# bupt-ai-cz/HIAST

Measured on AMD Instinct MI355X. Metric: self-training images/sec (fwd+bwd+pseudo-label) at 1024x512, higher is better.
Workload: dtype fp16

## Files before the change

hiast_amd/csrc/common.h:

```cpp
#pragma once
#include <hip/hip_runtime.h>
#include <hip/hip_bf16.h>
#include <hip/hip_fp16.h>
#include <stdint.h>

#include <type_traits>

#include "../../include/hiast_hip.h"

#define HIAST_WAVE 64

#define HIAST_CHECK_LAUNCH()                         \
    do {                                             \
        hipError_t e__ = hipGetLastError();          \
        if (e__ != hipSuccess) return (int)e__;      \
    } while (0)

static inline int hiast_fmt_planes(int fmt) { return fmt == HIAST_FMT_SPLIT_BF16 ? 2 : 1; }
static inline int hiast_fmt_ok(int fmt) { return fmt == HIAST_FMT_BF16 || fmt == HIAST_FMT_SPLIT_BF16 || fmt == HIAST_FMT_FP16; }

int hiast_cu_count();
int hiast_grid_cus();

namespace hiast {

template <class F>
static inline bool for_class_count(int C, F&& f)
{
    switch (C) {
        case 19: f(std::integral_constant<int, 19>{}); return true;
        case 16: f(std::integral_constant<int, 16>{}); return true;
        case 9:  f(std::integral_constant<int, 9>{});  return true;
        case 2:  f(std::integral_constant<int, 2>{});  return true;
        default: return false;
    }
}

typedef __attribute__((ext_vector_type(8))) __bf16 h_bf16x8;
typedef __attribute__((ext_vector_type(8))) _Float16 h_f16x8;
typedef __attribute__((ext_vector_type(4))) float h_f32x4;
typedef __attribute__((ext_vector_type(16))) float h_f32x16;

typedef __attribute__((address_space(3))) void* h_lds_ptr;
__device__ __forceinline__ void h_dma16(__amdgpu_buffer_rsrc_t rs, unsigned char* lds, int voff, int soff)
{
    __builtin_amdgcn_raw_ptr_buffer_load_lds(rs, (h_lds_ptr)lds, 16, voff, soff, 0, 0);
}
__device__ __forceinline__ int h_lds_off(int row, int chunk) { return row * 128 + ((chunk ^ ((row >> 1) & 7)) << 4); }

#ifndef HIAST_NT
#define HIAST_NT 1
#endif
__device__ __forceinline__ void h_store_f32(float* p, float v)
{
#if HIAST_NT
    __builtin_nontemporal_store(v, p);
#else
    *p = v;
#endif
}
typedef unsigned int h_u32x4 __attribute__((ext_vector_type(4)));
__device__ __forceinline__ void h_store16(void* p, unsigned a, unsigned b, unsigned c, unsigned d)
{
#if HIAST_NT
    __builtin_nontemporal_store((h_u32x4){a, b, c, d}, reinterpret_cast<h_u32x4*>(p));
#else
    *reinterpret_cast<uint4*>(p) = make_uint4(a, b, c, d);
#endif
}
__device__ __forceinline__ void h_store16(void* p, unsigned a, unsigned b, unsigned c, unsigned d, bool nt)
{
#if HIAST_NT
    if (nt) {
        __builtin_nontemporal_store((h_u32x4){a, b, c, d}, reinterpret_cast<h_u32x4*>(p));
        return;
    }
#endif
    *reinterpret_cast<uint4*>(p) = make_uint4(a, b, c, d);
}
#ifndef H_NT_MIN_MIB
#define H_NT_MIN_MIB 64
#endif
constexpr long long H_NT_MIN_BYTES = (long long)H_NT_MIN_MIB << 20;
#ifndef HIAST_NT_OUT
#define HIAST_NT_OUT 0
#endif
__device__ __forceinline__ void h_store16_out(void* p, unsigned a, unsigned b, unsigned c, unsigned d)
{
    h_store16(p, a, b, c, d, HIAST_NT_OUT != 0);
}
__device__ __forceinline__ void h_store_f32_out(float* p, float v)
{
#if HIAST_NT_OUT
    __builtin_nontemporal_store(v, p);
#else
    *p = v;
#endif
}
#ifndef HIAST_NT_RES
#define HIAST_NT_RES 0
#endif
__device__ __forceinline__ uint4 h_load16_once(const void* p)
{
#if HIAST_NT_RES
    const h_u32x4 v = __builtin_nontemporal_load(reinterpret_cast<const h_u32x4*>(p));
    return make_uint4(v.x, v.y, v.z, v.w);
#else
    return *reinterpret_cast<const uint4*>(p);
#endif
}

template <bool F16>
struct H16;

template <>
struct H16<false> {
    static __device__ __forceinline__ float lo(unsigned w) { return __uint_as_float(w << 16); }
    static __device__ __forceinline__ float hi(unsigned w) { return __uint_as_float(w & 0xFFFF0000u); }
    static __device__ __forceinline__ float dec(unsigned short h) { return __uint_as_float((unsigned)h << 16); }
    static __device__ __forceinline__ unsigned short enc(float v) { return __bfloat16_as_ushort(__float2bfloat16(v)); }
    static __device__ __forceinline__ unsigned pack(float a, float b) { return (unsigned)enc(a) | ((unsigned)enc(b) << 16); }
    template <class V>
    static __device__ __forceinline__ h_f32x4 mfma16(const V& a, const V& b, h_f32x4 c)
    {
        return __builtin_amdgcn_mfma_f32_16x16x32_bf16(__builtin_bit_cast(h_bf16x8, a), __builtin_bit_cast(h_bf16x8, b), c, 0, 0, 0);
    }
    template <class V>
    static __device__ __forceinline__ h_f32x16 mfma32(const V& a, const V& b, h_f32x16 c)
    {
        return __builtin_amdgcn_mfma_f32_32x32x16_bf16(__builtin_bit_cast(h_bf16x8, a), __builtin_bit_cast(h_bf16x8, b), c, 0, 0, 0);
    }
// ... 100 lines not shown
```

hiast_amd/csrc/conv_launch.h:

```cpp
#pragma once
#include <stdlib.h>

#include "common.h"

namespace hiast {

struct IGeo {
    int H, W, Ho, Wo, stride, dil;
};

}

struct ConvLaunch {
    const void* x = nullptr;
    const void* wp = nullptr;
    void* y = nullptr;
    const void* res = nullptr;
    const void* res_gate = nullptr;
    int gate_mask = 0;
    const float* gamma = nullptr;
    const float* beta = nullptr;
    const float* mean = nullptr;
    const float* var = nullptr;
    float eps = 0.0f;
    int relu = 0;
    int64_t M = 0;
    int K = 0, N = 0, taps = 1;
    hiast::IGeo geo = {0, 0, 0, 0, 1, 1};
    int fmt = HIAST_FMT_BF16;
    int out_f32 = 0;
    float* stats = nullptr;
    int stats_rows = 0;
    int stats_mode = 0;
    hipStream_t st = nullptr;

    int planes() const { return hiast_fmt_planes(fmt); }
    bool f16() const { return fmt == HIAST_FMT_FP16; }
};

enum class ConvFamily { XCONV, XCONV2, TILE_F16, TILE };

struct ConvRoute {
    ConvFamily family = ConvFamily::TILE;
    int BN = 0, BM = 0;
    bool half9 = false;
    int rows = 0;
};

static inline int conv_panel_streams(int64_t M, int NG, int panel_rows)
{
    static const int env_cus = [] { const char* e = getenv("HIAST_XCONV_CUS"); const int v = e ? atoi(e) : 0; return v >= 8 && v <= 256 ? v : 0; }();
    const long long npanel = (M + panel_rows - 1) / panel_rows;
    long long streams = (env_cus ? env_cus : hiast_grid_cus()) / NG / 8 * 8;
    if (streams < 8) streams = 8;
    if (streams > npanel) streams = (npanel + 7) / 8 * 8;
    return (int)streams;
}

ConvRoute ig_route(const ConvLaunch& c);
int hiast_igemm_launch(const ConvLaunch& c);
int hiast_igemm_launch_f16(const ConvLaunch& c, const ConvRoute& r);
int hiast_xconv_ok(const ConvLaunch& c);
int hiast_xconv_stats_rows(int64_t M, int N);
int hiast_xconv_launch(const ConvLaunch& c, const ConvRoute& r);
int hiast_xconv2_ok(const ConvLaunch& c);
int hiast_xconv2_launch(const ConvLaunch& c);
int hiast_gemm_nt_launch(const void* x, const float* w, void* y, int64_t M, int K, int N, int dtype, hipStream_t st);
```

hiast_amd/csrc/igemm.hip:

```cpp
#include "igemm_kernel.h"

namespace hiast {

template <int PL>
__device__ __forceinline__ size_t ig_wp_elem(int n, int t, int k, int taps, int KO)
{
    const size_t row = ((size_t)n * taps + t) * PL * KO;
    return PL == 2 ? row + (size_t)(k >> 5) * 64 + (k & 31) : row + k;
}

template <int PL, bool F16 = false>
__global__ __launch_bounds__(256) void pack_conv_weight_kernel(const float* __restrict__ w,
                                                               unsigned short* __restrict__ wp,
                                                               unsigned short* __restrict__ wpt, int N, int K, int taps,
                                                               int mode)
{
    const long long idx = (long long)blockIdx.x * 256 + threadIdx.x;
    if (idx >= (long long)N * taps * K) return;
    const int k = (int)(idx % K);
    const int t = (int)((idx / K) % taps);
    const int n = (int)(idx / ((long long)K * taps));
    const float v = w[((size_t)n * K + k) * taps + t];
    unsigned short h, l = 0;
    if (F16) h = H16<true>::enc(v);
// ... 122 lines not shown
__global__ __launch_bounds__(256) void from_planes_kernel(const unsigned short* __restrict__ p, float* __restrict__ x,
                                                          long long M, int C)
{
    const long long total8 = M * C / 8;
    for (long long i = (long long)blockIdx.x * 256 + threadIdx.x; i < total8; i += (long long)gridDim.x * 256) {
        const long long m = (i * 8) / C;
        const int c = (int)((i * 8) - m * C);
        const unsigned short* src = p + ig_elem<2>((size_t)m, c, C);
        const uint4 h = *reinterpret_cast<const uint4*>(src), l = *reinterpret_cast<const uint4*>(src + 32);
        const unsigned wh[4] = {h.x, h.y, h.z, h.w}, wl[4] = {l.x, l.y, l.z, l.w};
        float v[8];
#pragma unroll
        for (int q = 0; q < 4; ++q) {
            v[2 * q] = __uint_as_float(wh[q] << 16) + __uint_as_float(wl[q] << 16);
            v[2 * q + 1] = __uint_as_float(wh[q] & 0xFFFF0000u) + __uint_as_float(wl[q] & 0xFFFF0000u);
        }
        reinterpret_cast<float4*>(x)[2 * i] = make_float4(v[0], v[1], v[2], v[3]);
        reinterpret_cast<float4*>(x)[2 * i + 1] = make_float4(v[4], v[5], v[6], v[7]);
    }
}

}

struct IgEnv {
    int half;
    int bn;
    int ragged_off;
    int cosched0;
};
static const IgEnv& ig_env()
{
    static const IgEnv env = [] {
        IgEnv e;
        const char* v = getenv("HIAST_IGEMM_HALF");
        e.half = v ? (atoi(v) != 0) : -1;
        v = getenv("HIAST_IGEMM_BN");
        const int bn = v ? atoi(v) : 0;
        e.bn = (bn == 64 || bn == 128 || bn == 256) ? bn : 0;
        e.ragged_off = getenv("HIAST_IGEMM_RAGGED") != nullptr;
        v = getenv("HIAST_IGEMM_COSCHED");
        e.cosched0 = v && atoi(v) != 0;
        return e;
    }();
    return env;
}
static thread_local int ig_cosched_tls = -1, ig_half_tls = -1;
extern "C" int hiast_igemm_set_half(int v)
{
    const int prev = ig_half_tls;
    ig_half_tls = v < 0 ? -1 : (v != 0);
    return prev;
}
extern "C" int hiast_igemm_set_cosched(int on)
{
    const int prev = ig_cosched_tls;
    ig_cosched_tls = on < 0 ? -1 : (on != 0);
    return prev;
}
static int ig_half_forced() { return ig_half_tls >= 0 ? ig_half_tls : ig_env().half; }
static int ig_cosched() { return ig_cosched_tls >= 0 ? ig_cosched_tls : ig_env().cosched0; }

#ifndef IG_HALF_AUTO
#define IG_HALF_BLOCKS(M, N) ((((M) + 255) / 256) * (((N) % 256 == 0) ? (N) / 256 : (N) / 128))
#define IG_HALF_AUTO(M, K, N) (IG_HALF_BLOCKS(M, N) <= 64 || (IG_HALF_BLOCKS(M, N) <= 128 && !ig_cosched()))
#endif
static int ig_half_tile(int64_t M, int K, int N, int taps, int out_f32)
{
    if (taps != 1 || out_f32 || N % 128 != 0 || M < 4096) return 0;
    if (ig_half_forced() >= 0) return ig_half_forced();
    return IG_HALF_AUTO(M, K, N);
}
static int ig_half_tile9(int64_t M, int N, int PL, bool bn_relu_only)
{
    if (PL != 2 || !bn_relu_only || N % 128 != 0 || M < 4096) return 0;
    if (ig_half_forced() >= 0) return ig_half_forced();
    return IG_HALF_AUTO(M, 0, N);
}

ConvRoute ig_route(const ConvLaunch& c)
{
    ConvRoute r;
    if (c.stats_mode != 2 && hiast_xconv_ok(c)) {
        r.family = ConvFamily::XCONV;
        r.rows = hiast_xconv_stats_rows(c.M, c.N);
        return r;
    }
    if (c.stats_mode == 0 && !c.f16() && hiast_xconv2_ok(c)) {
        r.family = ConvFamily::XCONV2;
        return r;
    }
    r.family = c.f16() ? ConvFamily::TILE_F16 : ConvFamily::TILE;
    r.BN = (c.N % 256 == 0) ? 256 : ((c.N % 128 == 0) ? 128 : 64);
    const bool plain = !c.mean && !c.gamma && !c.res && !c.relu && !c.res_gate && c.stats_mode == 0;
    if (plain && !c.out_f32 && r.BN == 128 && c.N > 512 && !ig_env().ragged_off) r.BN = 256;
    if (const int v = ig_env().bn) {
        if (c.N % v == 0) r.BN = v;
    }
    r.half9 = c.taps == 9 && !c.out_f32 && c.geo.stride == 1 &&
              ig_half_tile9(c.M, c.N, c.planes(), c.mean && c.relu && !c.res && !c.res_gate && c.stats_mode == 0) != 0;
    const bool half = r.half9 || (c.geo.stride >= 0 && ig_half_tile(c.M, c.K, c.N, c.taps, c.out_f32) != 0);
    if (half) r.BN = 128;
    r.BM = half ? 128 : hiast::IG_BM;
    r.rows = (int)((c.M + r.BM - 1) / r.BM);
    return r;
}

int hiast_igemm_launch(const ConvLaunch& in)
{
    ConvLaunch c = in;
    if (c.stats_mode != 2) c.stats_mode = c.stats ? 1 : 0;
    const int H = c.geo.H, W = c.geo.W, stride = c.geo.stride, dil = c.geo.dil;
    if (!hiast_fmt_ok(c.fmt)) return HIAST_E_RANGE;
    const int planes = c.planes();
    if (c.stats_mode == 2) {
        if (!c.stats || !c.res || !c.mean || !c.var || planes != 1 || c.out_f32 || c.relu || c.res_gate || c.N % 8) return HIAST_E_RANGE;
    } else {
        if (c.stats && (planes != 1 || c.out_f32 || c.res || c.relu)) return HIAST_E_RANGE;
        if ((c.stats || c.res_gate) && c.mean) return HIAST_E_RANGE;
    }
    if (c.res_gate && (planes != 1 || !c.res || c.relu || c.out_f32 || (!c.gate_mask && (((uintptr_t)c.res_gate) & 15)))) return HIAST_E_RANGE;
    if (!c.x || !c.wp || !c.y || (c.mean && !c.var)) return HIAST_E_ARG;
    if (c.M <= 0 || c.K <= 0 || c.N <= 0) return HIAST_E_ARG;
    if ((planes != 1 && planes != 2) || (c.taps != 1 && c.taps != 9)) return HIAST_E_RANGE;
    if ((c.K * planes) % 64 != 0 || c.N % 64 != 0 || c.M > (1ll << 31) - 512) return HIAST_E_RANGE;
    if (c.out_f32 && c.res) return HIAST_E_RANGE;
    if ((((uintptr_t)c.x) | ((uintptr_t)c.wp) | ((uintptr_t)c.y) | ((uintptr_t)c.res)) & 15) return HIAST_E_RANGE;
    c.geo = {0, 0, 0, 0, 1, 1};
    size_t in_pix = (size_t)c.M;
    if (c.taps != 1 && stride == -2) {
        if (H <= 0 || W <= 0 || dil != 1 || planes != 1 || c.out_f32) return HIAST_E_ARG;
        const int Hs = (H - 1) / 2 + 1, Ws = (W - 1) / 2 + 1;
        if (c.M % ((int64_t)H * W) != 0) return HIAST_E_ARG;
        c.geo = {Hs, Ws, H, W, -2, 1};
        in_pix = (size_t)(c.M / ((int64_t)H * W)) * Hs * Ws;
    } else if (c.taps != 1) {
        if (H <= 0 || W <= 0 || stride <= 0 || dil <= 0) return HIAST_E_ARG;
        const int Ho = (H - 1) / stride + 1, Wo = (W - 1) / stride + 1;
        if (c.M % ((int64_t)Ho * Wo) != 0) return HIAST_E_ARG;
        c.geo = {H, W, Ho, Wo, stride, dil};
        in_pix = (size_t)(c.M / ((int64_t)Ho * Wo)) * H * W;
    }
    if (in_pix * planes * c.K * 2 >= (1ull << 31) || (size_t)c.N * c.taps * planes * c.K * 2 >= (1ull << 31)) return HIAST_E_RANGE;
    const ConvRoute r = ig_route(c);
    if (c.stats_mode != 0 && c.stats_rows != r.rows) return HIAST_E_ARG;
    switch (r.family) {
    case ConvFamily::XCONV: return hiast_xconv_launch(c, r);
    case ConvFamily::XCONV2: return hiast_xconv2_launch(c);
    case ConvFamily::TILE_F16: return hiast_igemm_launch_f16(c, r);
    case ConvFamily::TILE: break;
    }
    if (planes == 2) return c.out_f32 ? launch_igemm_t<2, true>(c, r) : launch_igemm_t<2, false>(c, r);
    return c.out_f32 ? launch_igemm_t<1, true>(c, r) : launch_igemm_t<1, false>(c, r);
}

extern "C" int hiast_igemm_dgrad_bn_stats(const void* dy, const void* wpt, void* da, int B, int H, int W, int Cin, int Cout,
                                          int taps, int dil, const void* bn_x, const float* gamma, const float* beta,
                                          const float* save_mean, const float* save_invstd, float* partial, int partial_rows,
                                          int fmt, hiast_stream_t stream)
{
    if (fmt != HIAST_FMT_BF16 && fmt != HIAST_FMT_FP16) return HIAST_E_RANGE;
    if (B <= 0 || H <= 0 || W <= 0) return HIAST_E_ARG;
    if (!bn_x || !save_mean || !save_invstd || !partial) return HIAST_E_ARG;
    if ((((uintptr_t)save_mean) | ((uintptr_t)save_invstd) | ((uintptr_t)gamma) | ((uintptr_t)beta)) & 15) return HIAST_E_RANGE;
    ConvLaunch c;
    c.x = dy; c.wp = wpt; c.y = da; c.res = bn_x;
    c.gamma = gamma; c.beta = beta; c.mean = save_mean; c.var = save_invstd;
    c.M = (int64_t)B * H * W; c.K = Cin; c.N = Cout; c.taps = taps;
// ... 267 lines not shown
```

hiast_amd/csrc/xconv.hip:

```cpp
#include <hip/hip_bf16.h>
#include <stdlib.h>

#include "conv_launch.h"

namespace hiast {

constexpr int XC_PANEL = 64;
constexpr int XC_STAGES = 3;
constexpr int XC_COLS = 512;

__device__ __forceinline__ h_bf16x8 xc_lds_read(unsigned addr)
{
    h_bf16x8 v;
    asm volatile("ds_read_b128 %0, %1" : "=v"(v) : "v"(addr));
    return v;
}
__device__ __forceinline__ void xc_lds_wait(h_bf16x8& a, h_bf16x8& b)
{
    asm volatile("s_waitcnt lgkmcnt(0)" : "+v"(a), "+v"(b));
}

__device__ __forceinline__ int xc_chan(int g, int b, int r) { return (b >> 1) * 32 + g * 8 + (b & 1) * 4 + r; }

template <int KC, bool BN, bool RES, bool RELU, bool GATE, bool STATS, bool F16 = false>
__global__ __launch_bounds__(512) void xconv_kernel(const unsigned short* __restrict__ X,
                                                    const unsigned short* __restrict__ Wp,
                                                    const float* __restrict__ gamma, const float* __restrict__ beta,
                                                    const float* __restrict__ mean, const float* __restrict__ var,
                                                    float eps, const unsigned short* __restrict__ R,
                                                    const unsigned char* __restrict__ Rg,
                                                    unsigned short* __restrict__ Y, int M, int N,
                                                    float* __restrict__ stats)
{
    constexpr int SL = KC / 64;
    constexpr int KS = KC / 32;
    constexpr int STAGE = XC_PANEL * KC * 2;
    __shared__ __attribute__((aligned(1024))) unsigned char smem[XC_STAGES * STAGE];
    __shared__ float s_sc[XC_COLS], s_sh[XC_COLS];

    const int tid = threadIdx.x, lane = tid & 63;
    const int wave = __builtin_amdgcn_readfirstlane(tid >> 6);
    const int g = lane >> 4, px = lane & 15;
    const int NG = N / XC_COLS;
    const int xcd = blockIdx.x & 7, slot = blockIdx.x >> 3;
    const int cg = slot % NG;
    const int nstream = (int)gridDim.x / NG;
    const int stream = (slot / NG) * 8 + xcd;
    const int n0 = cg * XC_COLS + wave * 64;
    const int npanel = (M + XC_PANEL - 1) / XC_PANEL;

    h_bf16x8 wr[4][KS];
#pragma unroll
    for (int b = 0; b < 4; ++b) {
        const unsigned short* wrow = Wp + (size_t)(n0 + xc_chan(px >> 2, b, px & 3)) * KC + g * 8;
#pragma unroll
        for (int s = 0; s < KS; ++s) wr[b][s] = *reinterpret_cast<const h_bf16x8*>(wrow + s * 32);
    }
#pragma unroll
    for (int b = 0; b < 4; ++b)
#pragma unroll
        for (int s = 0; s < KS; ++s) asm volatile("" : "+v"(wr[b][s]));
    if (BN) {
        for (int c = tid; c < XC_COLS; c += 512) {
            const int n = cg * XC_COLS + c;
            const float sc = (gamma ? gamma[n] : 1.0f) * (1.0f / sqrtf(var[n] + eps));
            s_sc[c] = sc;
            s_sh[c] = fmaf(-mean[n], sc, beta ? beta[n] : 0.0f);
        }
        __syncthreads();
    }

    constexpr int OOB = (int)0x80000000;
    const __amdgpu_buffer_rsrc_t xrs = __builtin_amdgcn_make_buffer_rsrc((void*)X, 0, (int)((size_t)M * KC * 2), 0x00020000);
    const int drow = wave * 8 + (lane >> 3);
    const int dchunk = ((lane & 7) ^ ((drow >> 1) & 7)) * 16;
    auto issue = [&](int p, int st) {
        const int m = p * XC_PANEL + drow;
        const int voff = (p < npanel && m < M) ? (int)((size_t)m * KC * 2) + dchunk : OOB;
        unsigned char* base = smem + st * STAGE + wave * 1024;
#pragma unroll
        for (int j = 0; j < SL; ++j) h_dma16(xrs, base + j * (XC_PANEL * 128), voff, j * 128);
    };

    const unsigned lds_base = (unsigned)(size_t)smem;
    float st1[STATS ? 16 : 1], st2[STATS ? 16 : 1];
#pragma unroll
    for (int q = 0; q < (STATS ? 16 : 1); ++q) { st1[q] = 0.f; st2[q] = 0.f; }

    issue(stream, 0);
    issue(stream + nstream, 1);
    int it = 0;
    for (int p = stream; p < npanel; p += nstream, ++it) {
        const int st = it % XC_STAGES;
        constexpr int NRES = RES ? (GATE ? 8 : 4) : 0;
        if (it == 0) asm volatile("s_waitcnt vmcnt(%0)\n\ts_barrier" ::"n"(SL) : "memory");
        else asm volatile("s_waitcnt vmcnt(%0)\n\ts_barrier" ::"n"(SL + 8 + NRES) : "memory");
        uint4 rres[RES ? 2 : 1][2];
        unsigned rgate[GATE ? 2 : 1][2];
        auto load_res = [&](int half) {
#pragma unroll
            for (int t = 0; t < 2; ++t) {
                const int m = p * XC_PANEL + half * 32 + t * 16 + px;
                const size_t row = (size_t)(m < M ? m : 0) * N + n0 + g * 8;
                rres[t][0] = h_load16_once(R + row);
                rres[t][1] = h_load16_once(R + row + 32);
                if (GATE) {
                    const unsigned char* gp = Rg + (size_t)(m < M ? m : 0) * (N >> 3) + ((n0 + g * 8) >> 3);
                    rgate[t][0] = gp[0];
                    rgate[t][1] = gp[4];
                }
            }
        };
        if (RES) load_res(0);
        issue(p + 2 * nstream, (it + 2) % XC_STAGES);
#pragma unroll
        for (int half = 0; half < 2; ++half) {
            if (RES && half == 1) load_res(1);
            h_f32x4 acc[2][4];
#pragma unroll
            for (int a = 0; a < 2; ++a)
#pragma unroll
                for (int b = 0; b < 4; ++b) acc[a][b] = (h_f32x4){0.f, 0.f, 0.f, 0.f};
            auto frag = [&](int s, int a) {
                return xc_lds_read(lds_base + (unsigned)(st * STAGE + (s >> 1) * (XC_PANEL * 128) +
                                                         h_lds_off(half * 32 + a * 16 + px, (s & 1) * 4 + g)));
            };
            constexpr bool DB = !(STATS || (BN && RES));
            h_bf16x8 xa[DB ? 2 : 1][2];
            xa[0][0] = frag(0, 0);
            xa[0][1] = frag(0, 1);
            xc_lds_wait(xa[0][0], xa[0][1]);
#pragma unroll
            for (int s = 0; s < KS; ++s) {
                constexpr int one = DB ? 1 : 0;
                if (DB && s + 1 < KS) {
                    xa[(s + 1) & one][0] = frag(s + 1, 0);
                    xa[(s + 1) & one][1] = frag(s + 1, 1);
                }
#pragma unroll
                for (int a = 0; a < 2; ++a)
#pragma unroll
                    for (int b = 0; b < 4; ++b)
                        acc[a][b] = H16<F16>::mfma16(wr[b][s], xa[s & one][a], acc[a][b]);
                if (s + 1 < KS) {
                    if (!DB) {
                        xa[0][0] = frag(s + 1, 0);
                        xa[0][1] = frag(s + 1, 1);
                    }
                    xc_lds_wait(xa[(s + 1) & one][0], xa[(s + 1) & one][1]);
                }
            }
#pragma unroll
            for (int a = 0; a < 2; ++a) {
                const int m = p * XC_PANEL + half * 32 + a * 16 + px;
                const bool ok = m < M;
                const size_t row = (size_t)(ok ? m : 0) * N + n0 + g * 8;
                const uint4 r0 = rres[RES ? a : 0][0], r1 = rres[RES ? a : 0][1];
                const unsigned gate0 = GATE ? rgate[GATE ? a : 0][0] : 0xFFu;
                const unsigned gate1 = GATE ? rgate[GATE ? a : 0][1] : 0xFFu;
                float o[16];
#pragma unroll
                for (int b = 0; b < 4; ++b)
#pragma unroll
                    for (int r = 0; r < 4; ++r) o[(b >> 1) * 8 + (b & 1) * 4 + r] = acc[a][b][r];
                if (BN) {
#pragma unroll
                    for (int hh = 0; hh < 2; ++hh) {
                        const int c = wave * 64 + hh * 32 + g * 8;
#pragma unroll
                        for (int q = 0; q < 8; q += 4) {
                            const float4 sc = *reinterpret_cast<const float4*>(&s_sc[c + q]);
                            const float4 sh = *reinterpret_cast<const float4*>(&s_sh[c + q]);
                            o[hh * 8 + q] = fmaf(o[hh * 8 + q], sc.x, sh.x);
                            o[hh * 8 + q + 1] = fmaf(o[hh * 8 + q + 1], sc.y, sh.y);
                            o[hh * 8 + q + 2] = fmaf(o[hh * 8 + q + 2], sc.z, sh.z);
                            o[hh * 8 + q + 3] = fmaf(o[hh * 8 + q + 3], sc.w, sh.w);
                        }
                    }
                }
                if (RES) {
                    const unsigned w0[4] = {r0.x, r0.y, r0.z, r0.w}, w1[4] = {r1.x, r1.y, r1.z, r1.w};
#pragma unroll
                    for (int q = 0; q < 4; ++q) {
                        float a0 = H16<F16>::lo(w0[q]), a1 = H16<F16>::hi(w0[q]);
                        float b0 = H16<F16>::lo(w1[q]), b1 = H16<F16>::hi(w1[q]);
                        if (GATE) {
                            a0 = ((gate0 >> (2 * q)) & 1u) ? a0 : 0.f;
                            a1 = ((gate0 >> (2 * q + 1)) & 1u) ? a1 : 0.f;
                            b0 = ((gate1 >> (2 * q)) & 1u) ? b0 : 0.f;
                            b1 = ((gate1 >> (2 * q + 1)) & 1u) ? b1 : 0.f;
                        }
                        o[2 * q] += a0;
                        o[2 * q + 1] += a1;
                        o[8 + 2 * q] += b0;
                        o[8 + 2 * q + 1] += b1;
                    }
                }
                if (RELU) {
#pragma unroll
                    for (int q = 0; q < 16; ++q) o[q] = o[q] > 0.f ? o[q] : 0.f;
                }
                unsigned pk[8];
                if (STATS && F16) {
#pragma unroll
                    for (int q = 0; q < 8; ++q) {
                        pk[q] = H16<F16>::pack(o[2 * q], o[2 * q + 1]);
                        if (ok) {
                            const float v0 = H16<F16>::lo(pk[q]), v1 = H16<F16>::hi(pk[q]);
                            st1[2 * q] += v0; st2[2 * q] = fmaf(v0, v0, st2[2 * q]);
                            st1[2 * q + 1] += v1; st2[2 * q + 1] = fmaf(v1, v1, st2[2 * q + 1]);
                        }
                        __builtin_amdgcn_sched_barrier(0);
                    }
                } else {
#pragma unroll
                    for (int q = 0; q < 8; ++q) pk[q] = H16<F16>::pack(o[2 * q], o[2 * q + 1]);
                    if (STATS && ok) {
#pragma unroll
                        for (int q = 0; q < 8; ++q) {
                            const float v0 = H16<F16>::lo(pk[q]), v1 = H16<F16>::hi(pk[q]);
                            st1[2 * q] += v0; st2[2 * q] = fmaf(v0, v0, st2[2 * q]);
                            st1[2 * q + 1] += v1; st2[2 * q + 1] = fmaf(v1, v1, st2[2 * q + 1]);
                        }
                    }
                }
                if (ok) {
                    h_store16_out(Y + row, pk[0], pk[1], pk[2], pk[3]);
                    h_store16_out(Y + row + 32, pk[4], pk[5], pk[6], pk[7]);
                }
            }
        }
    }
    if (STATS) {
#pragma unroll
        for (int q = 0; q < 16; ++q) {
#pragma unroll
            for (int o = 1; o < 16; o <<= 1) {
                st1[q] += __shfl_xor(st1[q], o, 64);
                st2[q] += __shfl_xor(st2[q], o, 64);
            }
        }
        if (px == 0) {
            float* d = stats + ((size_t)stream * N + n0 + g * 8) * 2;
#pragma unroll
            for (int q = 0; q < 8; ++q) {
                d[2 * q] = st1[q];
                d[2 * q + 1] = st2[q];
                d[64 + 2 * q] = st1[8 + q];
                d[64 + 2 * q + 1] = st2[8 + q];
            }
        }
    }
}

}

int hiast_xconv_ok(const ConvLaunch& c)
{
    const char* env = getenv("HIAST_XCONV");
    const bool has_bn = c.mean != nullptr, has_res = c.res != nullptr;
    if ((env && atoi(env) == 0) || c.planes() != 1 || c.taps != 1 || c.out_f32) return 0;
    if (c.K != 256 || c.N % hiast::XC_COLS != 0 || c.N > 2048) return 0;
    if (c.res_gate && (!c.gate_mask || !has_res || c.relu)) return 0;
    if (has_bn && has_res && !c.relu) return 0;
    if (c.stats_mode == 1 && (has_res || c.relu || has_bn)) return 0;
    if (c.M < 4096) return 0;
    return 1;
}

int hiast_xconv_stats_rows(int64_t M, int N)
{
    return conv_panel_streams(M, N / hiast::XC_COLS, hiast::XC_PANEL);
}

int hiast_xconv_launch(const ConvLaunch& c, const ConvRoute& r)
{
    using namespace hiast;
    const dim3 grid((unsigned)(r.rows * (c.N / XC_COLS)));
#define XK(BNF, RESF, RELUF, GATEF, STATSF, F16)                                                                      \
    hipLaunchKernelGGL((xconv_kernel<256, BNF, RESF, RELUF, GATEF, STATSF, F16>), grid, dim3(512), 0, c.st,           \
                       (const unsigned short*)c.x, (const unsigned short*)c.wp, c.gamma, c.beta, c.mean, c.var, c.eps, \
                       (const unsigned short*)c.res, (const unsigned char*)c.res_gate, (unsigned short*)c.y, (int)c.M, c.N, \
                       c.stats)
#define XL(BNF, RESF, RELUF, GATEF, STATSF)                                                                          \
    do {                                                                                                             \
        if (c.f16()) XK(BNF, RESF, RELUF, GATEF, STATSF, true);                                                      \
        else XK(BNF, RESF, RELUF, GATEF, STATSF, false);                                                             \
    } while (0)
    const bool bn = c.mean != nullptr;
    if (c.stats) { XL(false, false, false, false, true); }
    else if (c.res_gate) { XL(false, true, false, true, false); }
    else if (c.res) {
        if (bn) { if (c.relu) XL(true, true, true, false, false); else return HIAST_E_RANGE; }
        else { if (c.relu) XL(false, true, true, false, false); else XL(false, true, false, false, false); }
    } else {
        if (bn) { if (c.relu) XL(true, false, true, false, false); else XL(true, false, false, false, false); }
        else { if (c.relu) XL(false, false, true, false, false); else XL(false, false, false, false, false); }
    }
#undef XL
#undef XK
    HIAST_CHECK_LAUNCH();
    return 0;
}
```

hiast_amd/csrc/xconv_bs.hip:

```cpp
#include <hip/hip_bf16.h>
#include <stdlib.h>

#include "common.h"

namespace hiast {

constexpr int XB_PANEL = 64;
constexpr int XB_STAGES = 3;
constexpr int XB_COLS = 256;
constexpr int XB_KC = 256;

template <int IDX>
__device__ __forceinline__ h_bf16x8 xb_lds_read_i(unsigned addr)
{
    h_bf16x8 v;
    asm volatile("ds_read_b128 %0, %1 offset:%2" : "=v"(v) : "v"(addr), "i"(IDX * 2048));
    return v;
}
__device__ __forceinline__ h_bf16x8 xb_lds_read(unsigned addr, int idx)
{
    switch (idx) {
    case 1: return xb_lds_read_i<1>(addr);
    case 2: return xb_lds_read_i<2>(addr);
    case 3: return xb_lds_read_i<3>(addr);
    case 4: return xb_lds_read_i<4>(addr);
    case 5: return xb_lds_read_i<5>(addr);
    case 6: return xb_lds_read_i<6>(addr);
    case 7: return xb_lds_read_i<7>(addr);
    case 8: return xb_lds_read_i<8>(addr);
    case 9: return xb_lds_read_i<9>(addr);
    case 10: return xb_lds_read_i<10>(addr);
    case 11: return xb_lds_read_i<11>(addr);
    case 12: return xb_lds_read_i<12>(addr);
    case 13: return xb_lds_read_i<13>(addr);
    case 14: return xb_lds_read_i<14>(addr);
    case 15: return xb_lds_read_i<15>(addr);
    default: return xb_lds_read_i<0>(addr);
    }
}
__device__ __forceinline__ void xb_lds_wait(h_bf16x8& a, h_bf16x8& b)
{
    asm volatile("s_waitcnt lgkmcnt(0)" : "+v"(a), "+v"(b));
}

template <bool F16>
__global__ __launch_bounds__(512) void xconv_gated_bnstat_kernel(
    const unsigned short* __restrict__ X, const unsigned short* __restrict__ Wp, const unsigned short* __restrict__ R,
    const unsigned char* __restrict__ Rg, const unsigned short* __restrict__ BX, const unsigned char* __restrict__ BM,
    const float* __restrict__ bmean, const float* __restrict__ binvstd, unsigned short* __restrict__ Y, int M, int N,
    float* __restrict__ stats)
{
    constexpr int SL = XB_KC / 64;
    constexpr int KS = XB_KC / 32;
    constexpr int STAGE = XB_PANEL * XB_KC * 2;
    __shared__ __attribute__((aligned(1024))) unsigned char smem[XB_STAGES * STAGE];

    const int tid = threadIdx.x, lane = tid & 63;
    const int wave = __builtin_amdgcn_readfirstlane(tid >> 6);
    const int g = lane >> 4, px = lane & 15;
    const int NG = N / XB_COLS;
    const int xcd = blockIdx.x & 7, slot = blockIdx.x >> 3;
    const int cg = slot % NG;
    const int nstream = (int)gridDim.x / NG;
    const int stream = (slot / NG) * 8 + xcd;
    const int n0 = cg * XB_COLS + wave * 32;
    const int npanel = (M + XB_PANEL - 1) / XB_PANEL;
    const int c0 = n0 + g * 8;

    h_bf16x8 wr[2][KS];
#pragma unroll
    for (int b = 0; b < 2; ++b) {
        const unsigned short* wrow = Wp + (size_t)(n0 + (px >> 2) * 8 + b * 4 + (px & 3)) * XB_KC + g * 8;
#pragma unroll
        for (int s = 0; s < KS; ++s) wr[b][s] = *reinterpret_cast<const h_bf16x8*>(wrow + s * 32);
    }
#pragma unroll
    for (int b = 0; b < 2; ++b)
#pragma unroll
        for (int s = 0; s < KS; ++s) asm volatile("" : "+v"(wr[b][s]));

    constexpr int OOB = (int)0x80000000;
    const __amdgpu_buffer_rsrc_t xrs = __builtin_amdgcn_make_buffer_rsrc((void*)X, 0, (int)((size_t)M * XB_KC * 2), 0x00020000);
    const int drow = wave * 8 + (lane >> 3);
    const int dchunk = ((lane & 7) ^ ((drow >> 1) & 7)) * 16;
    auto issue = [&](int p, int st) {
        const int m = p * XB_PANEL + drow;
        const int voff = (p < npanel && m < M) ? (int)((size_t)m * XB_KC * 2) + dchunk : OOB;
        unsigned char* base = smem + st * STAGE + wave * 1024;
#pragma unroll
        for (int j = 0; j < SL; ++j) h_dma16(xrs, base + j * (XB_PANEL * 128), voff, j * 128);
    };
    const unsigned lds_base = (unsigned)(size_t)smem;
    float st1[8], st2[8];
#pragma unroll
    for (int q = 0; q < 8; ++q) { st1[q] = 0.f; st2[q] = 0.f; }

    struct Rows {
        uint4 res[4], bx[4];
        unsigned gate[4], bm[4];
    };
    Rows ring[2];
    auto load_rows = [&](Rows& r, int p) {
#pragma unroll
        for (int t = 0; t < 4; ++t) {
            const int m = p * XB_PANEL + t * 16 + px;
            const size_t mr = (size_t)((p < npanel && m < M) ? m : 0);
            r.res[t] = h_load16_once(R + mr * N + c0);
            r.gate[t] = Rg[mr * (N >> 3) + (c0 >> 3)];
            r.bx[t] = h_load16_once(BX + mr * N + c0);
            r.bm[t] = BM[mr * (N >> 3) + (c0 >> 3)];
        }
    };
    auto panel = [&](int p, int it, const Rows& cur, Rows& nxt) {
        const int st = it % XB_STAGES;
        if (it == 0) asm volatile("s_waitcnt vmcnt(%0)\n\ts_barrier" ::"n"(SL + 16) : "memory");
        else asm volatile("s_waitcnt vmcnt(%0)\n\ts_barrier" ::"n"(SL + 4) : "memory");
        load_rows(nxt, p + nstream);
        issue(p + 2 * nstream, (it + 2) % XB_STAGES);
        const unsigned fbase = lds_base + (unsigned)(st * STAGE) + (unsigned)h_lds_off(px, g);
#pragma unroll
        for (int half = 0; half < 2; ++half) {
            h_f32x4 acc[2][2];
#pragma unroll
            for (int a = 0; a < 2; ++a)
#pragma unroll
                for (int b = 0; b < 2; ++b) acc[a][b] = (h_f32x4){0.f, 0.f, 0.f, 0.f};
            auto frag = [&](int s, int a) {
                return xb_lds_read((s & 1) ? fbase ^ 64u : fbase, 4 * (s >> 1) + 2 * half + a);
            };
            h_bf16x8 xa[2][2];
            xa[0][0] = frag(0, 0);
            xa[0][1] = frag(0, 1);
            xb_lds_wait(xa[0][0], xa[0][1]);
#pragma unroll
            for (int s = 0; s < KS; ++s) {
                if (s + 1 < KS) {
                    xa[(s + 1) & 1][0] = frag(s + 1, 0);
                    xa[(s + 1) & 1][1] = frag(s + 1, 1);
                }
#pragma unroll
                for (int a = 0; a < 2; ++a)
#pragma unroll
                    for (int b = 0; b < 2; ++b) acc[a][b] = H16<F16>::mfma16(wr[b][s], xa[s & 1][a], acc[a][b]);
                if (s + 1 < KS) xb_lds_wait(xa[(s + 1) & 1][0], xa[(s + 1) & 1][1]);
            }
#pragma unroll
            for (int a = 0; a < 2; ++a) {
                const int t = 2 * half + a;
                const int m = p * XB_PANEL + t * 16 + px;
                const bool ok = m < M;
                const unsigned w0[4] = {cur.res[t].x, cur.res[t].y, cur.res[t].z, cur.res[t].w};
                const unsigned xw[4] = {cur.bx[t].x, cur.bx[t].y, cur.bx[t].z, cur.bx[t].w};
                const unsigned gate = cur.gate[t], bm = cur.bm[t];
                unsigned pk[4];
#pragma unroll
                for (int q = 0; q < 4; ++q) {
                    float o0 = acc[a][q >> 1][2 * (q & 1)], o1 = acc[a][q >> 1][2 * (q & 1) + 1];
                    o0 += ((gate >> (2 * q)) & 1u) ? H16<F16>::lo(w0[q]) : 0.f;
                    o1 += ((gate >> (2 * q + 1)) & 1u) ? H16<F16>::hi(w0[q]) : 0.f;
                    pk[q] = H16<F16>::pack(o0, o1);
                    if (ok) {
                        const float g0 = ((bm >> (2 * q)) & 1u) ? H16<F16>::lo(pk[q]) : 0.f;
                        const float g1 = ((bm >> (2 * q + 1)) & 1u) ? H16<F16>::hi(pk[q]) : 0.f;
                        st1[2 * q] += g0;
                        st2[2 * q] = fmaf(g0, H16<F16>::lo(xw[q]), st2[2 * q]);
                        st1[2 * q + 1] += g1;
                        st2[2 * q + 1] = fmaf(g1, H16<F16>::hi(xw[q]), st2[2 * q + 1]);
                    }
                }
                if (ok) h_store16_out(Y + (size_t)m * N + c0, pk[0], pk[1], pk[2], pk[3]);
            }
        }
    };

    issue(stream, 0);
    issue(stream + nstream, 1);
    load_rows(ring[0], stream);
    for (int p = stream, it = 0; p < npanel; p += 2 * nstream, it += 2) {
        panel(p, it, ring[0], ring[1]);
        if (p + nstream >= npanel) break;
        panel(p + nstream, it + 1, ring[1], ring[0]);
    }
#pragma unroll
    for (int q = 0; q < 8; ++q) {
#pragma unroll
        for (int o = 1; o < 16; o <<= 1) {
            st1[q] += __shfl_xor(st1[q], o, 64);
            st2[q] += __shfl_xor(st2[q], o, 64);
        }
    }
    if (px == 0) {
        float* d = stats + ((size_t)stream * N + c0) * 2;
#pragma unroll
        for (int q = 0; q < 8; ++q) {
            const float mu = bmean[c0 + q], is = binvstd[c0 + q];
            d[2 * q] = st1[q];
            d[2 * q + 1] = is * (st2[q] - mu * st1[q]);
        }
    }
}

static int xb_blocks(int64_t M, int N)
{
    const int NG = N / XB_COLS;
    const long long npanel = (M + XB_PANEL - 1) / XB_PANEL;
    long long streams = hiast_grid_cus() / NG / 8 * 8;
    if (streams < 8) streams = 8;
    if (streams > npanel) streams = (npanel + 7) / 8 * 8;
    return (int)(streams * NG);
}

// ... 36 lines not shown
```

Before: 143.7.

## Extend fused 1x1 xconv kernel to K=512 with narrower wave columns

Generalizes the persistent 1x1-conv (xconv) kernel so K=512 layers can use it. For K=512 it keeps one 32 KiB LDS stage per panel by halving the panel rows and using 32 output columns per wave. It also adds triple-buffered LDS fragment reads with counted waits and loads residual rows one panel ahead. This routes K=512 convs away from the generic igemm path, at the cost of more template instantiations and a register/occupancy profile that may not suit every shape.

```diff
diff --git a/hiast_amd/csrc/common.h b/hiast_amd/csrc/common.h
--- a/hiast_amd/csrc/common.h
+++ b/hiast_amd/csrc/common.h
@@ -47,6 +47,35 @@
     __builtin_amdgcn_raw_ptr_buffer_load_lds(rs, (h_lds_ptr)lds, 16, voff, soff, 0, 0);
 }
 __device__ __forceinline__ int h_lds_off(int row, int chunk) { return row * 128 + ((chunk ^ ((row >> 1) & 7)) << 4); }
+
+template <int IDX>
+__device__ __forceinline__ h_bf16x8 h_lds_read_2k_i(unsigned addr)
+{
+    h_bf16x8 v;
+    asm volatile("ds_read_b128 %0, %1 offset:%2" : "=v"(v) : "v"(addr), "i"(IDX * 2048));
+    return v;
+}
+__device__ __forceinline__ h_bf16x8 h_lds_read_2k(unsigned addr, int idx)
+{
+    switch (idx) {
+    case 1: return h_lds_read_2k_i<1>(addr);
+    case 2: return h_lds_read_2k_i<2>(addr);
+    case 3: return h_lds_read_2k_i<3>(addr);
+    case 4: return h_lds_read_2k_i<4>(addr);
+    case 5: return h_lds_read_2k_i<5>(addr);
+    case 6: return h_lds_read_2k_i<6>(addr);
+    case 7: return h_lds_read_2k_i<7>(addr);
+    case 8: return h_lds_read_2k_i<8>(addr);
+    case 9: return h_lds_read_2k_i<9>(addr);
+    case 10: return h_lds_read_2k_i<10>(addr);
+    case 11: return h_lds_read_2k_i<11>(addr);
+    case 12: return h_lds_read_2k_i<12>(addr);
+    case 13: return h_lds_read_2k_i<13>(addr);
+    case 14: return h_lds_read_2k_i<14>(addr);
+    case 15: return h_lds_read_2k_i<15>(addr);
+    default: return h_lds_read_2k_i<0>(addr);
+    }
+}
 
 #ifndef HIAST_NT
 #define HIAST_NT 1
diff --git a/hiast_amd/csrc/conv_launch.h b/hiast_amd/csrc/conv_launch.h
--- a/hiast_amd/csrc/conv_launch.h
+++ b/hiast_amd/csrc/conv_launch.h
@@ -61,7 +61,7 @@
 int hiast_igemm_launch(const ConvLaunch& c);
 int hiast_igemm_launch_f16(const ConvLaunch& c, const ConvRoute& r);
 int hiast_xconv_ok(const ConvLaunch& c);
-int hiast_xconv_stats_rows(int64_t M, int N);
+int hiast_xconv_stats_rows(int64_t M, int K, int N);
 int hiast_xconv_launch(const ConvLaunch& c, const ConvRoute& r);
 int hiast_xconv2_ok(const ConvLaunch& c);
 int hiast_xconv2_launch(const ConvLaunch& c);
diff --git a/hiast_amd/csrc/igemm.hip b/hiast_amd/csrc/igemm.hip
--- a/hiast_amd/csrc/igemm.hip
+++ b/hiast_amd/csrc/igemm.hip
@@ -228,7 +228,7 @@
     ConvRoute r;
     if (c.stats_mode != 2 && hiast_xconv_ok(c)) {
         r.family = ConvFamily::XCONV;
-        r.rows = hiast_xconv_stats_rows(c.M, c.N);
+        r.rows = hiast_xconv_stats_rows(c.M, c.K, c.N);
         return r;
     }
     if (c.stats_mode == 0 && !c.f16() && hiast_xconv2_ok(c)) {
diff --git a/hiast_amd/csrc/xconv.hip b/hiast_amd/csrc/xconv.hip
--- a/hiast_amd/csrc/xconv.hip
+++ b/hiast_amd/csrc/xconv.hip
@@ -5,9 +5,10 @@
 
 namespace hiast {
 
-constexpr int XC_PANEL = 64;
 constexpr int XC_STAGES = 3;
-constexpr int XC_COLS = 512;
+constexpr int XC_STAGE = 32768;
+constexpr int xc_cw(int K) { return K == 512 ? 32 : 64; }
+constexpr int xc_panel(int K) { return XC_STAGE / (K * 2); }
 
 __device__ __forceinline__ h_bf16x8 xc_lds_read(unsigned addr)
 {
@@ -15,14 +16,15 @@
     asm volatile("ds_read_b128 %0, %1" : "=v"(v) : "v"(addr));
     return v;
 }
+template <int LEFT = 0>
 __device__ __forceinline__ void xc_lds_wait(h_bf16x8& a, h_bf16x8& b)
 {
-    asm volatile("s_waitcnt lgkmcnt(0)" : "+v"(a), "+v"(b));
+    asm volatile("s_waitcnt lgkmcnt(%2)" : "+v"(a), "+v"(b) : "n"(LEFT));
 }
 
 __device__ __forceinline__ int xc_chan(int g, int b, int r) { return (b >> 1) * 32 + g * 8 + (b & 1) * 4 + r; }
 
-template <int KC, bool BN, bool RES, bool RELU, bool GATE, bool STATS, bool F16 = false>
+template <int KC, int CW, bool BN, bool RES, bool RELU, bool GATE, bool STATS, bool F16 = false>
 __global__ __launch_bounds__(512) void xconv_kernel(const unsigned short* __restrict__ X,
                                                     const unsigned short* __restrict__ Wp,
                                                     const float* __restrict__ gamma, const float* __restrict__ beta,
@@ -34,7 +36,14 @@
 {
     constexpr int SL = KC / 64;
     constexpr int KS = KC / 32;
+    constexpr int XC_PANEL = xc_panel(KC);
+    constexpr int XC_COLS = 8 * CW;
     constexpr int STAGE = XC_PANEL * KC * 2;
+    constexpr int NT = CW / 16;
+    constexpr int NQ = CW / 32;
+    constexpr int OC = 8 * NQ;
+    constexpr int HALVES = XC_PANEL / 32;
+    static_assert(STAGE == XC_STAGE && (CW == 64 || CW == 32) && (HALVES == 1 || HALVES == 2), "panel = one 32 KiB stage");
     __shared__ __attribute__((aligned(1024))) unsigned char smem[XC_STAGES * STAGE];
     __shared__ float s_sc[XC_COLS], s_sh[XC_COLS];
 
@@ -46,18 +55,18 @@
     const int cg = slot % NG;
     const int nstream = (int)gridDim.x / NG;
     const int stream = (slot / NG) * 8 + xcd;
-    const int n0 = cg * XC_COLS + wave * 64;
+    const int n0 = cg * XC_COLS + wave * CW;
     const int npanel = (M + XC_PANEL - 1) / XC_PANEL;
 
-    h_bf16x8 wr[4][KS];
-#pragma unroll
-    for (int b = 0; b < 4; ++b) {
+    h_bf16x8 wr[NT][KS];
+#pragma unroll
+    for (int b = 0; b < NT; ++b) {
         const unsigned short* wrow = Wp + (size_t)(n0 + xc_chan(px >> 2, b, px & 3)) * KC + g * 8;
 #pragma unroll
         for (int s = 0; s < KS; ++s) wr[b][s] = *reinterpret_cast<const h_bf16x8*>(wrow + s * 32);
     }
 #pragma unroll
-    for (int b = 0; b < 4; ++b)
+    for (int b = 0; b < NT; ++b)
 #pragma unroll
         for (int s = 0; s < KS; ++s) asm volatile("" : "+v"(wr[b][s]));
     if (BN) {
@@ -71,83 +80,126 @@
     }
 
     constexpr int OOB = (int)0x80000000;
+    constexpr int RG = XC_PANEL / 8;
+    constexpr int NDMA = SL * RG / 8;
+    static_assert(NDMA == 4, "the counted waits below assume 4 DMA instructions per wave and panel");
     const __amdgpu_buffer_rsrc_t xrs = __builtin_amdgcn_make_buffer_rsrc((void*)X, 0, (int)((size_t)M * KC * 2), 0x00020000);
-    const int drow = wave * 8 + (lane >> 3);
+    const int drg = RG == 8 ? wave : wave % RG, dsl = RG == 8 ? 0 : (wave / RG) * NDMA;
+    const int drow = drg * 8 + (lane >> 3);
     const int dchunk = ((lane & 7) ^ ((drow >> 1) & 7)) * 16;
     auto issue = [&](int p, int st) {
         const int m = p * XC_PANEL + drow;
         const int voff = (p < npanel && m < M) ? (int)((size_t)m * KC * 2) + dchunk : OOB;
-        unsigned char* base = smem + st * STAGE + wave * 1024;
-#pragma unroll
-        for (int j = 0; j < SL; ++j) h_dma16(xrs, base + j * (XC_PANEL * 128), voff, j * 128);
+        unsigned char* base = smem + st * STAGE + drg * 1024;
+#pragma unroll
+        for (int j = 0; j < NDMA; ++j) h_dma16(xrs, base + (dsl + j) * (XC_PANEL * 128), voff, (dsl + j) * 128);
     };
 
     const unsigned lds_base = (unsigned)(size_t)smem;
-    float st1[STATS ? 16 : 1], st2[STATS ? 16 : 1];
-#pragma unroll
-    for (int q = 0; q < (STATS ? 16 : 1); ++q) { st1[q] = 0.f; st2[q] = 0.f; }
+    float st1[STATS ? OC : 1], st2[STATS ? OC : 1];
+#pragma unroll
+    for (int q = 0; q < (STATS ? OC : 1); ++q) { st1[q] = 0.f; st2[q] = 0.f; }
+
+    auto load_rows = [&](int m0, auto& rr, auto& gg) {
+#pragma unroll
+        for (int t = 0; t < 2; ++t) {
+            const int m = m0 + t * 16 + px;
+            const size_t row = (size_t)(m < M ? m : 0) * N + n0 + g * 8;
+            rr[t][0] = h_load16_once(R + row);
+            if (NQ == 2) rr[t][1] = h_load16_once(R + row + 32);
+            if (GATE) {
+                const unsigned char* gp = Rg + (size_t)(m < M ? m : 0) * (N >> 3) + ((n0 + g * 8) >> 3);
+                gg[t][0] = gp[0];
+                if (NQ == 2) gg[t][1] = gp[4];
+            }
+        }
+    };
+    constexpr bool AHEAD = RES && HALVES == 1;
+    uint4 rnext[AHEAD ? 2 : 1][2];
+    unsigned gnext[AHEAD && GATE ? 2 : 1][2];
+    if (AHEAD) load_rows(stream * XC_PANEL, rnext, gnext);
 
     issue(stream, 0);
     issue(stream + nstream, 1);
     int it = 0;
     for (int p = stream; p < npanel; p += nstream, ++it) {
         const int st = it % XC_STAGES;
-        constexpr int NRES = RES ? (GATE ? 8 : 4) : 0;
-        if (it == 0) asm volatile("s_waitcnt vmcnt(%0)\n\ts_barrier" ::"n"(SL) : "memory");
-        else asm volatile("s_waitcnt vmcnt(%0)\n\ts_barrier" ::"n"(SL + 8 + NRES) : "memory");
+        constexpr int NRES = RES ? 2 * NQ * (GATE ? 2 : 1) : 0;
+        constexpr int NST = 2 * NQ;
+        if (it == 0) asm volatile("s_waitcnt vmcnt(%0)\n\ts_barrier" ::"n"(NDMA) : "memory");
+        else asm volatile("s_waitcnt vmcnt(%0)\n\ts_barrier" ::"n"(NDMA + HALVES * NST + (HALVES - 1) * NRES) : "memory");
         uint4 rres[RES ? 2 : 1][2];
         unsigned rgate[GATE ? 2 : 1][2];
-        auto load_res = [&](int half) {
+        auto load_res = [&](int half) { load_rows(p * XC_PANEL + half * 32, rres, rgate); };
+        if (AHEAD) {
 #pragma unroll
             for (int t = 0; t < 2; ++t) {
-                const int m = p * XC_PANEL + half * 32 + t * 16 + px;
-                const size_t row = (size_t)(m < M ? m : 0) * N + n0 + g * 8;
-                rres[t][0] = h_load16_once(R + row);
-                rres[t][1] = h_load16_once(R + row + 32);
-                if (GATE) {
-                    const unsigned char* gp = Rg + (size_t)(m < M ? m : 0) * (N >> 3) + ((n0 + g * 8) >> 3);
-                    rgate[t][0] = gp[0];
-                    rgate[t][1] = gp[4];
-                }
-            }
-        };
-        if (RES) load_res(0);
+                rres[t][0] = rnext[t][0];
+                if (GATE) rgate[t][0] = gnext[GATE ? t : 0][0];
+            }
+            load_rows((p + nstream) * XC_PANEL, rnext, gnext);
+        } else if (RES) load_res(0);
         issue(p + 2 * nstream, (it + 2) % XC_STAGES);
-#pragma unroll
-        for (int half = 0; half < 2; ++half) {
+        const unsigned fbase = lds_base + (unsigned)(st * STAGE) + (unsigned)h_lds_off(px, g);
+#pragma unroll
+        for (int half = 0; half < HALVES; ++half) {
             if (RES && half == 1) load_res(1);
-            h_f32x4 acc[2][4];
+            h_f32x4 acc[2][NT];
 #pragma unroll
             for (int a = 0; a < 2; ++a)
 #pragma unroll
-                for (int b = 0; b < 4; ++b) acc[a][b] = (h_f32x4){0.f, 0.f, 0.f, 0.f};
+                for (int b = 0; b < NT; ++b) acc[a][b] = (h_f32x4){0.f, 0.f, 0.f, 0.f};
             auto frag = [&](int s, int a) {
-                return xc_lds_read(lds_base + (unsigned)(st * STAGE + (s >> 1) * (XC_PANEL * 128) +
-                                                         h_lds_off(half * 32 + a * 16 + px, (s & 1) * 4 + g)));
+                if constexpr (HALVES == 1) return h_lds_read_2k((s & 1) ? fbase ^ 64u : fbase, 2 * (s >> 1) + a);
+                else return xc_lds_read(lds_base + (unsigned)(st * STAGE + (s >> 1) * (XC_PANEL * 128) +
+                                                              h_lds_off(half * 32 + a * 16 + px, (s & 1) * 4 + g)));
             };
-            constexpr bool DB = !(STATS || (BN && RES));
-            h_bf16x8 xa[DB ? 2 : 1][2];
-            xa[0][0] = frag(0, 0);
-            xa[0][1] = frag(0, 1);
-            xc_lds_wait(xa[0][0], xa[0][1]);
-#pragma unroll
-            for (int s = 0; s < KS; ++s) {
-                constexpr int one = DB ? 1 : 0;
-                if (DB && s + 1 < KS) {
-                    xa[(s + 1) & one][0] = frag(s + 1, 0);
-                    xa[(s + 1) & one][1] = frag(s + 1, 1);
-                }
-#pragma unroll
-                for (int a = 0; a < 2; ++a)
-#pragma unroll
-                    for (int b = 0; b < 4; ++b)
-                        acc[a][b] = H16<F16>::mfma16(wr[b][s], xa[s & one][a], acc[a][b]);
-                if (s + 1 < KS) {
-                    if (!DB) {
-                        xa[0][0] = frag(s + 1, 0);
-                        xa[0][1] = frag(s + 1, 1);
-                    }
-                    xc_lds_wait(xa[(s + 1) & one][0], xa[(s + 1) & one][1]);
+            constexpr bool DB = CW == 32 || !(STATS || (BN && RES));
+            if constexpr (CW == 32) {
+                h_bf16x8 xr[3][2];
+                xr[0][0] = frag(0, 0);
+                xr[0][1] = frag(0, 1);
+                xr[1][0] = frag(1, 0);
+                xr[1][1] = frag(1, 1);
+                xc_lds_wait<2>(xr[0][0], xr[0][1]);
+#pragma unroll
+                for (int s = 0; s < KS; ++s) {
+                    if (s + 2 < KS) {
+                        xr[(s + 2) % 3][0] = frag(s + 2, 0);
+                        xr[(s + 2) % 3][1] = frag(s + 2, 1);
+                    }
+#pragma unroll
+                    for (int a = 0; a < 2; ++a)
+#pragma unroll
+                        for (int b = 0; b < NT; ++b)
+                            acc[a][b] = H16<F16>::mfma16(wr[b][s], xr[s % 3][a], acc[a][b]);
+                    if (s + 2 < KS) xc_lds_wait<2>(xr[(s + 1) % 3][0], xr[(s + 1) % 3][1]);
+                    else if (s + 1 < KS) xc_lds_wait<0>(xr[(s + 1) % 3][0], xr[(s + 1) % 3][1]);
+                }
+            } else {
+                h_bf16x8 xa[DB ? 2 : 1][2];
+                xa[0][0] = frag(0, 0);
+                xa[0][1] = frag(0, 1);
+                xc_lds_wait(xa[0][0], xa[0][1]);
+#pragma unroll
+                for (int s = 0; s < KS; ++s) {
+                    constexpr int one = DB ? 1 : 0;
+                    if (DB && s + 1 < KS) {
+                        xa[(s + 1) & one][0] = frag(s + 1, 0);
+                        xa[(s + 1) & one][1] = frag(s + 1, 1);
+                    }
+#pragma unroll
+                    for (int a = 0; a < 2; ++a)
+#pragma unroll
+                        for (int b = 0; b < NT; ++b)
+                            acc[a][b] = H16<F16>::mfma16(wr[b][s], xa[s & one][a], acc[a][b]);
+                    if (s + 1 < KS) {
+                        if (!DB) {
+                            xa[0][0] = frag(s + 1, 0);
+                            xa[0][1] = frag(s + 1, 1);
+                        }
+                        xc_lds_wait(xa[(s + 1) & one][0], xa[(s + 1) & one][1]);
+                    }
                 }
             }
 #pragma unroll
@@ -155,18 +207,18 @@
                 const int m = p * XC_PANEL + half * 32 + a * 16 + px;
                 const bool ok = m < M;
                 const size_t row = (size_t)(ok ? m : 0) * N + n0 + g * 8;
-                const uint4 r0 = rres[RES ? a : 0][0], r1 = rres[RES ? a : 0][1];
+                const uint4 r0 = rres[RES ? a : 0][0], r1 = rres[RES ? a : 0][NQ - 1];
                 const unsigned gate0 = GATE ? rgate[GATE ? a : 0][0] : 0xFFu;
-                const unsigned gate1 = GATE ? rgate[GATE ? a : 0][1] : 0xFFu;
-                float o[16];
-#pragma unroll
-                for (int b = 0; b < 4; ++b)
+                const unsigned gate1 = GATE ? rgate[GATE ? a : 0][NQ - 1] : 0xFFu;
+                float o[OC];
+#pragma unroll
+                for (int b = 0; b < NT; ++b)
 #pragma unroll
                     for (int r = 0; r < 4; ++r) o[(b >> 1) * 8 + (b & 1) * 4 + r] = acc[a][b][r];
                 if (BN) {
 #pragma unroll
-                    for (int hh = 0; hh < 2; ++hh) {
-                        const int c = wave * 64 + hh * 32 + g * 8;
+                    for (int hh = 0; hh < NQ; ++hh) {
+                        const int c = wave * CW + hh * 32 + g * 8;
 #pragma unroll
                         for (int q = 0; q < 8; q += 4) {
                             const float4 sc = *reinterpret_cast<const float4*>(&s_sc[c + q]);
@@ -192,18 +244,20 @@
                         }
                         o[2 * q] += a0;
                         o[2 * q + 1] += a1;
-                        o[8 + 2 * q] += b0;
-                        o[8 + 2 * q + 1] += b1;
+                        if (NQ == 2) {
+                            o[OC - 8 + 2 * q] += b0;
+                            o[OC - 8 + 2 * q + 1] += b1;
+                        }
                     }
                 }
                 if (RELU) {
 #pragma unroll
-                    for (int q = 0; q < 16; ++q) o[q] = o[q] > 0.f ? o[q] : 0.f;
-                }
-                unsigned pk[8];
+                    for (int q = 0; q < OC; ++q) o[q] = o[q] > 0.f ? o[q] : 0.f;
+                }
+                unsigned pk[OC / 2];
                 if (STATS && F16) {
 #pragma unroll
-                    for (int q = 0; q < 8; ++q) {
+                    for (int q = 0; q < OC / 2; ++q) {
                         pk[q] = H16<F16>::pack(o[2 * q], o[2 * q + 1]);
                         if (ok) {
                             const float v0 = H16<F16>::lo(pk[q]), v1 = H16<F16>::hi(pk[q]);
@@ -214,10 +268,10 @@
                     }
                 } else {
 #pragma unroll
-                    for (int q = 0; q < 8; ++q) pk[q] = H16<F16>::pack(o[2 * q], o[2 * q + 1]);
+                    for (int q = 0; q < OC / 2; ++q) pk[q] = H16<F16>::pack(o[2 * q], o[2 * q + 1]);
                     if (STATS && ok) {
 #pragma unroll
-                        for (int q = 0; q < 8; ++q) {
+                        for (int q = 0; q < OC / 2; ++q) {
                             const float v0 = H16<F16>::lo(pk[q]), v1 = H16<F16>::hi(pk[q]);
                             st1[2 * q] += v0; st2[2 * q] = fmaf(v0, v0, st2[2 * q]);
                             st1[2 * q + 1] += v1; st2[2 * q + 1] = fmaf(v1, v1, st2[2 * q + 1]);
@@ -226,14 +280,14 @@
                 }
                 if (ok) {
                     h_store16_out(Y + row, pk[0], pk[1], pk[2], pk[3]);
-                    h_store16_out(Y + row + 32, pk[4], pk[5], pk[6], pk[7]);
+                    if (NQ == 2) h_store16_out(Y + row + 32, pk[OC / 2 - 4], pk[OC / 2 - 3], pk[OC / 2 - 2], pk[OC / 2 - 1]);
                 }
             }
         }
     }
     if (STATS) {
 #pragma unroll
-        for (int q = 0; q < 16; ++q) {
+        for (int q = 0; q < OC; ++q) {
 #pragma unroll
             for (int o = 1; o < 16; o <<= 1) {
                 st1[q] += __shfl_xor(st1[q], o, 64);
@@ -246,8 +300,10 @@
             for (int q = 0; q < 8; ++q) {
                 d[2 * q] = st1[q];
                 d[2 * q + 1] = st2[q];
-                d[64 + 2 * q] = st1[8 + q];
-                d[64 + 2 * q + 1] = st2[8 + q];
+                if (NQ == 2) {
+                    d[64 + 2 * q] = st1[OC - 8 + q];
+                    d[64 + 2 * q + 1] = st2[OC - 8 + q];
+                }
             }
         }
     }
@@ -260,7 +316,10 @@
     const char* env = getenv("HIAST_XCONV");
     const bool has_bn = c.mean != nullptr, has_res = c.res != nullptr;
     if ((env && atoi(env) == 0) || c.planes() != 1 || c.taps != 1 || c.out_f32) return 0;
-    if (c.K != 256 || c.N % hiast::XC_COLS != 0 || c.N > 2048) return 0;
+    if (c.K == 512) {
+        const char* e5 = getenv("HIAST_XCONV_K512");
+        if ((e5 && atoi(e5) == 0) || c.N % (8 * hiast::xc_cw(512)) != 0 || c.N < 2 * c.K) return 0;
+    } else if (c.K != 256 || c.N % (8 * hiast::xc_cw(256)) != 0 || c.N > 2048) return 0;
     if (c.res_gate && (!c.gate_mask || !has_res || c.relu)) return 0;
     if (has_bn && has_res && !c.relu) return 0;
     if (c.stats_mode == 1 && (has_res || c.relu || has_bn)) return 0;
@@ -268,24 +327,29 @@
     return 1;
 }
 
-int hiast_xconv_stats_rows(int64_t M, int N)
-{
-    return conv_panel_streams(M, N / hiast::XC_COLS, hiast::XC_PANEL);
+int hiast_xconv_stats_rows(int64_t M, int K, int N)
+{
+    return conv_panel_streams(M, N / (8 * hiast::xc_cw(K)), hiast::xc_panel(K));
 }
 
 int hiast_xconv_launch(const ConvLaunch& c, const ConvRoute& r)
 {
     using namespace hiast;
-    const dim3 grid((unsigned)(r.rows * (c.N / XC_COLS)));
-#define XK(BNF, RESF, RELUF, GATEF, STATSF, F16)                                                                      \
-    hipLaunchKernelGGL((xconv_kernel<256, BNF, RESF, RELUF, GATEF, STATSF, F16>), grid, dim3(512), 0, c.st,           \
+    const dim3 grid((unsigned)(r.rows * (c.N / (8 * xc_cw(c.K)))));
+#define XK(KC, BNF, RESF, RELUF, GATEF, STATSF, F16)                                                                  \
+    hipLaunchKernelGGL((xconv_kernel<KC, xc_cw(KC), BNF, RESF, RELUF, GATEF, STATSF, F16>), grid, dim3(512), 0, c.st, \
                        (const unsigned short*)c.x, (const unsigned short*)c.wp, c.gamma, c.beta, c.mean, c.var, c.eps, \
                        (const unsigned short*)c.res, (const unsigned char*)c.res_gate, (unsigned short*)c.y, (int)c.M, c.N, \
                        c.stats)
 #define XL(BNF, RESF, RELUF, GATEF, STATSF)                                                                          \
     do {                                                                                                             \
-        if (c.f16()) XK(BNF, RESF, RELUF, GATEF, STATSF, true);                                                      \
-        else XK(BNF, RESF, RELUF, GATEF, STATSF, false);                                                             \
+        if (c.K == 512) {                                                                                            \
+            if (c.f16()) XK(512, BNF, RESF, RELUF, GATEF, STATSF, true);                                             \
+            else XK(512, BNF, RESF, RELUF, GATEF, STATSF, false);                                                    \
+        } else {                                                                                                     \
+            if (c.f16()) XK(256, BNF, RESF, RELUF, GATEF, STATSF, true);                                             \
+            else XK(256, BNF, RESF, RELUF, GATEF, STATSF, false);                                                    \
+        }                                                                                                            \
     } while (0)
     const bool bn = c.mean != nullptr;
     if (c.stats) { XL(false, false, false, false, true); }
diff --git a/hiast_amd/csrc/xconv_bs.hip b/hiast_amd/csrc/xconv_bs.hip
--- a/hiast_amd/csrc/xconv_bs.hip
+++ b/hiast_amd/csrc/xconv_bs.hip
@@ -10,34 +10,6 @@
 constexpr int XB_COLS = 256;
 constexpr int XB_KC = 256;
 
-template <int IDX>
-__device__ __forceinline__ h_bf16x8 xb_lds_read_i(unsigned addr)
-{
-    h_bf16x8 v;
-    asm volatile("ds_read_b128 %0, %1 offset:%2" : "=v"(v) : "v"(addr), "i"(IDX * 2048));
-    return v;
-}
-__device__ __forceinline__ h_bf16x8 xb_lds_read(unsigned addr, int idx)
-{
-    switch (idx) {
-    case 1: return xb_lds_read_i<1>(addr);
-    case 2: return xb_lds_read_i<2>(addr);
-    case 3: return xb_lds_read_i<3>(addr);
-    case 4: return xb_lds_read_i<4>(addr);
-    case 5: return xb_lds_read_i<5>(addr);
-    case 6: return xb_lds_read_i<6>(addr);
-    case 7: return xb_lds_read_i<7>(addr);
-    case 8: return xb_lds_read_i<8>(addr);
-    case 9: return xb_lds_read_i<9>(addr);
-    case 10: return xb_lds_read_i<10>(addr);
-    case 11: return xb_lds_read_i<11>(addr);
-    case 12: return xb_lds_read_i<12>(addr);
-    case 13: return xb_lds_read_i<13>(addr);
-    case 14: return xb_lds_read_i<14>(addr);
-    case 15: return xb_lds_read_i<15>(addr);
-    default: return xb_lds_read_i<0>(addr);
-    }
-}
 __device__ __forceinline__ void xb_lds_wait(h_bf16x8& a, h_bf16x8& b)
 {
     asm volatile("s_waitcnt lgkmcnt(0)" : "+v"(a), "+v"(b));
@@ -126,7 +98,7 @@
 #pragma unroll
                 for (int b = 0; b < 2; ++b) acc[a][b] = (h_f32x4){0.f, 0.f, 0.f, 0.f};
             auto frag = [&](int s, int a) {
-                return xb_lds_read((s & 1) ? fbase ^ 64u : fbase, 4 * (s >> 1) + 2 * half + a);
+                return h_lds_read_2k((s & 1) ? fbase ^ 64u : fbase, 4 * (s >> 1) + 2 * half + a);
             };
             h_bf16x8 xa[2][2];
             xa[0][0] = frag(0, 0);
```

Result: slower. 139.7 (-2.8%).
